# aquaskyline/SOAPdenovo-Trans

Measured on AMD Instinct MI355X. Metric: pregraph k-mers hashed/sec, higher is better.
Workload: dtype u64

## Files before the change

### soapdenovo-trans_amd/csrc/sdt_sk_scatter_seq.cuh

```cuda
#pragma once
#include <hip/hip_runtime.h>
#include "sdt_kmer.cuh"
#include "sdt_table.cuh"
#include "sdt_superkmer.cuh"

using namespace sdt;

constexpr uint32_t SK_BLK = 128;
#ifndef SDT_SK_BLK2
#define SDT_SK_BLK2 1024
#endif
constexpr uint32_t SK_BLK2 = SDT_SK_BLK2;
constexpr uint32_t SK_DEAD = 0xFFFFFFFFu;

#ifdef SDT_SK_L2_LOG
extern __device__ unsigned long long *g_l2_log;
extern __device__ unsigned long long g_l2_log_cap;
__device__ inline void sk_log_alloc(uint32_t path, uint32_t end, uint32_t id)
{
	if (g_l2_log) {
		const unsigned long long at = atomicAdd(g_l2_log, 1ULL);
		if (at + 1 < g_l2_log_cap)
			g_l2_log[1 + at] = (1ULL << 63) | ((unsigned long long)path << 61) | ((unsigned long long)(threadIdx.x & 0x1FFF) << 48) |
			                   ((unsigned long long)(end & 0xFFFFFFu) << 24) | (unsigned long long)(id & 0xFFFFFFu);
	}
}
__device__ inline void sk_log_cursor(uint32_t kind, uint32_t lb, uint32_t chunk, uint32_t pos)
{
	if (g_l2_log) {
		const unsigned long long at = atomicAdd(g_l2_log, 1ULL);
		if (at + 1 < g_l2_log_cap)
			g_l2_log[1 + at] = (1ULL << 63) | (3ULL << 61) | ((unsigned long long)kind << 59) | ((unsigned long long)(blockIdx.x & 15u) << 55) |
			                   ((unsigned long long)(threadIdx.x & 1023u) << 45) | ((unsigned long long)(lb & 1023u) << 35) |
			                   ((unsigned long long)(pos > 31u ? 31u : pos) << 30) | (unsigned long long)(chunk & 0x3FFFFFFFu);
	}
}
#else
__device__ inline void sk_log_alloc(uint32_t, uint32_t, uint32_t) {}
__device__ inline void sk_log_cursor(uint32_t, uint32_t, uint32_t, uint32_t) {}
#endif

__device__ inline uint32_t sk_alloc_chunk(unsigned long long *s_blk, const SkPool &pool, uint32_t blk = SK_BLK)
{
	uint32_t got = 0;
	bool done = false;
	while (!done) {
		{
			const unsigned long long w = __hip_atomic_load(s_blk, __ATOMIC_RELAXED, __HIP_MEMORY_SCOPE_WORKGROUP);
			if ((uint32_t)w > (uint32_t)(w >> 32)) {
				__builtin_amdgcn_s_sleep(1);
				continue;
			}
		}
		const unsigned long long v = atomicAdd(s_blk, 1ULL);
		const uint32_t id = (uint32_t)v, end = (uint32_t)(v >> 32);
		if (id < end) {
			got = id;
			done = true;
			sk_log_alloc(0, end, id);
		} else if (id == end) {
			const uint32_t base = atomicAdd(pool.next, blk);
			atomicExch(s_blk, ((unsigned long long)(base + blk) << 32) | (unsigned long long)(base + 1u));
			got = base;
			done = true;
			sk_log_alloc(1, end, base);
		}
	}
	return got;
}

__device__ inline uint32_t sk_alloc_chunks(unsigned long long *s_blk, const SkPool &pool, uint32_t n, uint32_t blk)
{
	uint32_t got = SK_NOCHUNK;
	bool done = false;
	while (!done) {
		{
			const unsigned long long w = __hip_atomic_load(s_blk, __ATOMIC_RELAXED, __HIP_MEMORY_SCOPE_WORKGROUP);
			if ((uint32_t)w > (uint32_t)(w >> 32)) {
				__builtin_amdgcn_s_sleep(1);
				continue;
			}
		}
		const unsigned long long v = atomicAdd(s_blk, (unsigned long long)n);
		const uint32_t id = (uint32_t)v, end = (uint32_t)(v >> 32);
		if (id <= end && id + n <= end) {
			got = id;
			done = true;
		} else if (id <= end) {
			for (uint32_t x = id; x < end && x < pool.chunks; x++)
				pool.meta[x] = SK_DEAD;
			const uint32_t base = atomicAdd(pool.next, n + blk);
			atomicExch(s_blk, ((unsigned long long)(base + n + blk) << 32) | (unsigned long long)(base + n));
			got = base;
			done = true;
		}
	}
	return got;
}

__device__ inline void sk_retire_block(unsigned long long blk, const SkPool &pool)
{
	const uint32_t next = (uint32_t)blk, end = (uint32_t)(blk >> 32);
	for (uint32_t id = next; id < end && id < pool.chunks; id++)
		pool.meta[id] = SK_DEAD;
}

__device__ inline bool sk_reserve(unsigned long long *s_cur, unsigned long long *s_blk, uint32_t lb, uint32_t meta_bucket,
                                  uint32_t cap, const SkPool &pool, uint32_t *s_cnt, uint32_t &chunk, uint32_t &pos)
{
	bool done = false, ok = false;
	while (!done) {
		if ((uint32_t)__hip_atomic_load(&s_cur[lb], __ATOMIC_RELAXED, __HIP_MEMORY_SCOPE_WORKGROUP) > cap) {
			__builtin_amdgcn_s_sleep(1);
			continue;
		}
		const unsigned long long cur = atomicAdd(&s_cur[lb], 1ULL);
		pos = (uint32_t)cur;
		chunk = (uint32_t)(cur >> 32);
		if (pos < cap) {
			ok = chunk != SK_NOCHUNK;
			done = true;
			sk_log_cursor(0, lb, chunk, pos);
		} else if (pos == cap) {
			sk_log_cursor(1, lb, chunk, pos);
			uint32_t id = sk_alloc_chunk(s_blk, pool);
			if (id >= pool.chunks) {
				id = SK_NOCHUNK;
			} else {
				pool.meta[id] = meta_bucket | (cap << 24);
				atomicAdd(&s_cnt[lb], 1u);
			}
			atomicExch(&s_cur[lb], ((unsigned long long)id << 32) | 1ULL);
			chunk = id;
			pos = 0;
			ok = id != SK_NOCHUNK;
			done = true;
			sk_log_cursor(3, lb, id, 1);
		} else {
#if SDT_SK_L2_LOG >= 2
			sk_log_cursor(2, lb, chunk, pos);
#endif
		}
	}
	return ok;
}

template <int RW> __device__ inline void sk_store_record(uint64_t *dst, const uint64_t (&rec)[RW])
{
#pragma unroll
	for (int i = 0; i < RW; i++)
		dst[i] = rec[i];
}
template <int NW> __device__ inline void sk_store_record2(uint64_t *dst, const uint64_t (&rec)[SkFmt<NW>::REC_WORDS])
{
	if constexpr (SkFmt<NW>::REC2_STRIDE == 4 && SkFmt<NW>::REC_WORDS == 3) {
		ulonglong2 *d = reinterpret_cast<ulonglong2 *>(dst);
		d[0] = make_ulonglong2(rec[0], rec[1]);
		d[1] = make_ulonglong2(rec[2], 0ULL);
	} else {
		sk_store_record<SkFmt<NW>::REC_WORDS>(dst, rec);
	}
}
template <int RW> __device__ inline void sk_load_record(const uint64_t *src, uint64_t (&rec)[RW])
{
#pragma unroll
	for (int i = 0; i < RW; i++)
		rec[i] = src[i];
}


constexpr int SK_SEQ_TILE = 256;
constexpr int SK_SEQ_RUNCAP = 24;
constexpr int SK_SEQ_MAX_KMERS = 256;


template <int NW>
__device__ inline void sk_emit_run(const uint32_t *words, int rb_r, int len_r, int nk_r, int K, uint64_t read_ord, int j0, int n,
                                   uint32_t fb, unsigned long long *s_cur, unsigned long long *s_blk, const SkPool &pool,
                                   uint32_t *s_cnt, const Table<NW> &tbl, uint32_t &claimed, uint32_t &failed, uint32_t &done,
                                   uint32_t &emitted)
{
	constexpr int BW = SkFmt<NW>::BW, RW = SkFmt<NW>::REC_WORDS;
	const int hp = j0 > 0, hn = j0 + n < nk_r;
	const uint32_t l1 = fb >> SK_L2BITS, l2 = fb & (SK_NB2 - 1);
	uint32_t chunk, pos;
	if (sk_reserve(s_cur, s_blk, l1, l1, SK_CAP1, pool, s_cnt, chunk, pos)) {
		const int len = hp + n + K - 1 + hn, ps = rb_r + j0 - hp;
		uint64_t rec[RW];
		rec[0] = sk_header(read_ord, (uint32_t)j0, l2, n, hp, hn);
#pragma unroll
		for (int k = 0; k < BW; k++) {
			uint64_t wv = 0;
			if (32 * k < len) {
				wv = sk_stream_word(words, ps + 32 * k);
				const int keep = len - 32 * k;
				if (keep < 32)
					wv &= ~0ULL << (64 - 2 * keep);
			}
			rec[1 + k] = wv;
		}
		sk_store_record<RW>(pool.recs + ((size_t)chunk * SK_CAP1 + pos) * RW, rec);
		emitted += (uint32_t)n;
	} else if (!tbl.ent) {
		failed += (uint32_t)n;
	} else {
		for (int jj = j0; jj < j0 + n; jj++) {
			uint32_t prev, next;
			const Key<NW> key = chop_record<NW>(words, rb_r, len_r, jj, K, prev, next);
			const uint64_t ord = tbl.first ? (read_ord << 16) | (uint64_t)jj : ORD_NONE;
			if (!table_put<NW>(tbl, key, prev, next, claimed, ord))
				failed++;
			done++;
		}
	}
}

template <int NW, int W>
__global__ __launch_bounds__(SK_SEQ_TILE, NW == 1 ? 4 : 2) void k_sk_scatter_reads_seq(const uint32_t *__restrict__ packed, const uint64_t *__restrict__ offs,
                                                                      uint64_t nreads, int K, int m, int ncap, int max_tile_words, SkPool pool,
                                                                      unsigned long long *__restrict__ g_cursors, unsigned long long *__restrict__ g_blk,
                                                                      uint32_t *__restrict__ g_cnt, Table<NW> tbl, Stats *stats,
                                                                      uint64_t ord_base, uint64_t ord_stride)
{
	constexpr int TR = SK_SEQ_TILE;
	extern __shared__ uint32_t smem[];
	unsigned long long *s_cur = (unsigned long long *)smem;
	uint32_t *s_rb = (uint32_t *)(s_cur + SK_NB1);
	uint32_t *s_runs = s_rb + TR + 2;
	uint32_t *s_words = s_runs + TR * SK_SEQ_RUNCAP;
	__shared__ unsigned long long s_blk;
	__shared__ uint32_t s_cnt[SK_NB1];
	const int tid = threadIdx.x;
	for (int i = tid; i < SK_NB1; i += TR) {
		s_cur[i] = g_cursors[(size_t)blockIdx.x * SK_NB1 + i];
		s_cnt[i] = 0;
	}
	if (tid == 0)
		s_blk = g_blk[blockIdx.x];
	const uint64_t ntiles = (nreads + TR - 1) / TR;
	const uint32_t mmask = (1u << (2 * m)) - 1u;
	const int topsh = 2 * (m - 1);
	uint32_t claimed = 0, failed = 0, done = 0, emitted = 0;
#ifdef SDT_SK_TICKS
	unsigned long long cyc[4] = {0, 0, 0, 0}, t0 = wall_clock64(), t1;
#define SK_TICK(i) do { t1 = wall_clock64(); cyc[i] += t1 - t0; t0 = t1; } while (0)
#else
#define SK_TICK(i) do { } while (0)
#endif
	for (uint64_t tile = blockIdx.x; tile < ntiles; tile += gridDim.x) {
		const uint64_t r0 = tile * TR;
		const int nr = (int)((nreads - r0) < (uint64_t)TR ? (nreads - r0) : (uint64_t)TR);
		const uint64_t word0 = offs[r0] >> 4;
		int nwords = (int)(((offs[r0 + nr] + 15) >> 4) - word0) + TAIL_PAD;
		if (nwords > max_tile_words)
			nwords = max_tile_words;
		s_rb[tid] = (uint32_t)(offs[r0 + (tid < nr ? tid : nr)] - (word0 << 4));
		if (tid == 0)
			s_rb[TR] = (uint32_t)(offs[r0 + nr] - (word0 << 4));
		if (tid < LDS_LEAD)
			s_words[tid] = 0;
		for (int i = tid; i < nwords; i += TR)
			s_words[LDS_LEAD + i] = packed[word0 + i];
		__syncthreads();
		SK_TICK(0);
		const uint32_t *words = s_words + LDS_LEAD;
		const int rb_r = (int)s_rb[tid];
		const int len_r = tid < nr ? (int)s_rb[tid + 1] - rb_r : 0;
		const int nk_r = len_r >= K + 1 ? len_r - K + 1 : 0;
		const uint64_t read_ord = ord_base + (r0 + (uint64_t)tid) * ord_stride;
		uint32_t *runs = s_runs + tid * SK_SEQ_RUNCAP;
		int nrun = 0;
		if (nk_r > 0) {
			const int nhv = len_r - m + 1;
			uint32_t fw = sk_stream_mmer(words, rb_r, m) >> 2;
			uint32_t rc = (sk_rev2bit32(fw ^ 0xAAAAAAAAu) >> (32 - 2 * (m - 1))) << 2;
			int pb = rb_r + m - 1;
			auto next_hv = [&]() -> uint32_t {
				const uint32_t b = (words[pb >> 4] >> (30 - 2 * (pb & 15))) & 3u;
				pb++;
				fw = ((fw << 2) | b) & mmask;
				rc = (rc >> 2) | ((b ^ 2u) << topsh);
				return sk_mmer_hash(fw < rc ? fw : rc);
			};
			int j0 = 0;
			uint32_t fb0 = 0, pfb = 0;
			auto window = [&](int j, uint32_t mn) {
				const uint32_t fb = sk_final_bucket(sk_bucket_hash(mn));
				if (j == 0) {
					fb0 = fb;
				} else if (j - j0 >= ncap || fb != pfb) {
					if (nrun < SK_SEQ_RUNCAP)
						runs[nrun] = (fb0 << 6) | (uint32_t)(j - j0 - 1);
					else
						sk_emit_run<NW>(words, rb_r, len_r, nk_r, K, read_ord, j0, j - j0, fb0, s_cur, &s_blk, pool, s_cnt, tbl, claimed, failed, done, emitted);
					nrun++;
					j0 = j;
					fb0 = fb;
				}
				pfb = fb;
			};
			uint32_t h[W], nh[W];
#pragma clang loop unroll(full)
			for (int i = 0; i < W; i++)
				h[i] = next_hv();
#pragma clang loop unroll(full)
			for (int i = W - 2; i >= 0; i--)
				h[i] = h[i] < h[i + 1] ? h[i] : h[i + 1];
			int p = W;
			for (int jb = 0; jb < nk_r; jb += W) {
				window(jb, h[0]);
				uint32_t pre = 0xFFFFFFFFu;
#pragma clang loop unroll(full)
				for (int i = 1; i < W; i++) {
					const uint32_t x = p < nhv ? next_hv() : 0xFFFFFFFFu;
					p++;
					nh[i - 1] = x;
					pre = x < pre ? x : pre;
					if (jb + i < nk_r)
						window(jb + i, h[i] < pre ? h[i] : pre);
				}
				nh[W - 1] = p < nhv ? next_hv() : 0xFFFFFFFFu;
				p++;
				h[W - 1] = nh[W - 1];
#pragma clang loop unroll(full)
				for (int i = W - 2; i >= 0; i--)
					h[i] = nh[i] < h[i + 1] ? nh[i] : h[i + 1];
			}
			if (nrun < SK_SEQ_RUNCAP)
				runs[nrun] = (fb0 << 6) | (uint32_t)(nk_r - j0 - 1);
			else
				sk_emit_run<NW>(words, rb_r, len_r, nk_r, K, read_ord, j0, nk_r - j0, fb0, s_cur, &s_blk, pool, s_cnt, tbl, claimed, failed, done, emitted);
			nrun++;
		}
		SK_TICK(1);
		const int nlist = nrun < SK_SEQ_RUNCAP ? nrun : SK_SEQ_RUNCAP;
		for (int k = 0, jr = 0; k < nlist; k++) {
			const uint32_t e = runs[k];
			const int nr = (int)(e & 63u) + 1;
			sk_emit_run<NW>(words, rb_r, len_r, nk_r, K, read_ord, jr, nr, e >> 6, s_cur, &s_blk, pool, s_cnt, tbl, claimed, failed, done, emitted);
			jr += nr;
		}
		__syncthreads();
		SK_TICK(3);
	}
#undef SK_TICK
	for (int i = tid; i < SK_NB1; i += TR) {
		g_cursors[(size_t)blockIdx.x * SK_NB1 + i] = s_cur[i];
		if (s_cnt[i])
			atomicAdd(&g_cnt[i], s_cnt[i]);
	}
	if (tid == 0) {
		g_blk[blockIdx.x] = s_blk;
#ifdef SDT_SK_TICKS
		for (int i = 0; i < 4; i++)
			atomicAdd(&stats->sk_cyc1[i], cyc[i]);
#endif
	}
	if (done) {
		atomicAdd(&stats->kmers, (unsigned long long)done);
		atomicAdd(&stats->sk_direct, (unsigned long long)done);
	}
	if (claimed) atomicAdd(&stats->distinct, (unsigned long long)claimed);
	if (failed) atomicAdd(&stats->probe_fail, (unsigned long long)failed);
#pragma unroll
	for (int d = 32; d > 0; d >>= 1)
		emitted += __shfl_down(emitted, d);
	if ((tid & 63) == 0 && emitted)
		atomicAdd(&stats->sk_emitted, (unsigned long long)emitted);
}


struct SkSeqLaunch {
	const uint32_t *words;
	const uint64_t *offs;
	uint64_t nreads;
	int K, m, ncap, mtw;
	SkPool pool;
	unsigned long long *cursors, *blk;
	uint32_t *cnt;
	Stats *stats;
	uint64_t ord_base, ord_stride;
	unsigned max_wgs;
	int cu_count;
	hipStream_t stream;
};

template <int NW, int W> inline hipError_t sk_seq_launch_one(const SkSeqLaunch &a, const Table<NW> &tbl)
{
	const size_t smem = (size_t)SK_NB1 * 8 + (size_t)(SK_SEQ_TILE + 2) * 4 + (size_t)SK_SEQ_TILE * SK_SEQ_RUNCAP * 4 + (size_t)(LDS_LEAD + a.mtw) * 4;
	hipError_t e = hipFuncSetAttribute((const void *)k_sk_scatter_reads_seq<NW, W>, hipFuncAttributeMaxDynamicSharedMemorySize, (int)smem);
	if (e != hipSuccess) return e;
	int per_cu = 0;
	e = hipOccupancyMaxActiveBlocksPerMultiprocessor(&per_cu, k_sk_scatter_reads_seq<NW, W>, SK_SEQ_TILE, smem);
	if (e != hipSuccess) return e;
	uint64_t res = (uint64_t)(per_cu > 0 ? per_cu : 1) * (uint64_t)a.cu_count;
	if (res > a.max_wgs) res = a.max_wgs;
	const uint64_t nt = (a.nreads + SK_SEQ_TILE - 1) / SK_SEQ_TILE;
	const unsigned grid = (unsigned)(nt < res ? nt : res);
	hipLaunchKernelGGL((k_sk_scatter_reads_seq<NW, W>), dim3(grid), dim3(SK_SEQ_TILE), smem, a.stream, a.words, a.offs, a.nreads, a.K, a.m, a.ncap,
	                   a.mtw, a.pool, a.cursors, a.blk, a.cnt, tbl, a.stats, a.ord_base, a.ord_stride);
	return hipGetLastError();
}

hipError_t sk_seq_launch_nw1(int w, const SkSeqLaunch &a, const Table<1> &tbl);
hipError_t sk_seq_launch_nw2_lo(int w, const SkSeqLaunch &a, const Table<2> &tbl);
hipError_t sk_seq_launch_nw2_mid(int w, const SkSeqLaunch &a, const Table<2> &tbl);
hipError_t sk_seq_launch_nw2_hi(int w, const SkSeqLaunch &a, const Table<2> &tbl);
```

Before: 95.24 billion.

## Restructure super-k-mer walk with batched base loads and branchless run recording

Moves the minimizer window walk into a reusable helper that loads W bases at once from two LDS words per 16 bases, instead of one LDS read per base. Run boundaries are recorded branchlessly into an LDS list with an extra overflow slot, and a read is re-walked in segments when the list fills, rather than emitting overflow runs inline. The record packing in sk_emit_run now builds 32-bit halves from clamped word loads with masks, replacing the per-word stream-and-branch code. The extra per-thread LDS slot raises shared memory use and could lower occupancy, and the restart logic adds complexity for reads with many runs.

```diff
diff --git a/soapdenovo-trans_amd/csrc/sdt_sk_scatter_seq.cuh b/soapdenovo-trans_amd/csrc/sdt_sk_scatter_seq.cuh
--- a/soapdenovo-trans_amd/csrc/sdt_sk_scatter_seq.cuh
+++ b/soapdenovo-trans_amd/csrc/sdt_sk_scatter_seq.cuh
@@ -174,6 +174,116 @@
 constexpr int SK_SEQ_MAX_KMERS = 256;
 
 
+template <int W, class List>
+__host__ __device__ inline int sk_walk_list(const uint32_t *words, int rb, int nk, int m, int ncap, List &list)
+{
+	constexpr int NA = (W + 15) / 16, CAP = List::CAP;
+	const uint32_t mmask = (1u << (2 * m)) - 1u;
+	const int topsh = 2 * (m - 1);
+	const int ncm1 = ncap - 1;
+	uint32_t fw = sk_stream_mmer(words, rb, m) >> 2;
+	uint32_t rc = (sk_rev2bit32(fw ^ 0xAAAAAAAAu) >> (32 - 2 * (m - 1))) << 2;
+	int pb = rb + m - 1;
+	uint32_t a[NA], c[NA];
+	auto load = [&]() {
+		const int wi = pb >> 4, sh = 32 - 2 * (pb & 15);
+		uint32_t d[NA + 1];
+#pragma clang loop unroll(full)
+		for (int i = 0; i <= NA; i++)
+			d[i] = words[wi + i];
+#pragma clang loop unroll(full)
+		for (int i = 0; i < NA; i++) {
+			a[i] = (uint32_t)((((uint64_t)d[i] << 32) | d[i + 1]) >> sh);
+			c[i] = a[i] ^ 0xAAAAAAAAu;
+		}
+		pb += W;
+	};
+	auto hv = [&](int k) -> uint32_t {
+		const uint32_t b = (a[k >> 4] >> (30 - 2 * (k & 15))) & 3u;
+		const uint32_t bc = (c[k >> 4] >> (30 - 2 * (k & 15))) & 3u;
+		fw = ((fw << 2) | b) & mmask;
+		rc = (rc >> 2) | (bc << topsh);
+		return sk_mmer_hash(fw < rc ? fw : rc);
+	};
+	uint32_t h[W], nh[W];
+	load();
+#pragma clang loop unroll(full)
+	for (int i = 0; i < W; i++)
+		h[i] = hv(i);
+#pragma clang loop unroll(full)
+	for (int i = W - 2; i >= 0; i--)
+		h[i] = h[i] < h[i + 1] ? h[i] : h[i + 1];
+	int nm1 = -1, nrun = 0;
+	uint32_t pfb = sk_final_bucket(sk_bucket_hash(h[0]));
+	auto window = [&](uint32_t mn) {
+		const uint32_t fb = sk_final_bucket(sk_bucket_hash(mn));
+		const bool end = nm1 >= ncm1 || fb != pfb;
+		list.put(nrun < CAP ? nrun : CAP, (pfb << 6) | (uint32_t)nm1);
+		nrun += end ? 1 : 0;
+		nm1 = end ? 0 : nm1 + 1;
+		pfb = fb;
+	};
+	for (int jb = 0; jb < nk && nrun < CAP; jb += W) {
+		const int nv = nk - jb;
+		uint32_t pre = 0xFFFFFFFFu;
+		if (nv > W) {
+			load();
+			window(h[0]);
+#pragma clang loop unroll(full)
+			for (int i = 1; i < W; i++) {
+				const uint32_t x = hv(i - 1);
+				nh[i - 1] = x;
+				pre = x < pre ? x : pre;
+				window(h[i] < pre ? h[i] : pre);
+			}
+			nh[W - 1] = hv(W - 1);
+			h[W - 1] = nh[W - 1];
+#pragma clang loop unroll(full)
+			for (int i = W - 2; i >= 0; i--)
+				h[i] = nh[i] < h[i + 1] ? nh[i] : h[i + 1];
+		} else {
+			if (nv > 1)
+				load();
+			window(h[0]);
+#pragma clang loop unroll(full)
+			for (int i = 1; i < W; i++) {
+				if (i < nv) {
+					const uint32_t x = hv(i - 1);
+					pre = x < pre ? x : pre;
+					window(h[i] < pre ? h[i] : pre);
+				}
+			}
+		}
+	}
+	list.put(nrun < CAP ? nrun : CAP, (pfb << 6) | (uint32_t)nm1);
+	nrun++;
+	return nrun < CAP ? nrun : CAP;
+}
+
+template <int W, class List, class Run, class Tick>
+__host__ __device__ inline void sk_walk_read(const uint32_t *words, int rb, int nk, int m, int ncap, List &list, Run &&run, Tick &&tick)
+{
+	int js = 0;
+	do {
+		const int nl = sk_walk_list<W>(words, rb + js, nk - js, m, ncap, list);
+		tick(1);
+		for (int k = 0; k < nl; k++) {
+			const uint32_t e = list.get(k);
+			const int n = (int)(e & 63u) + 1;
+			run(js, n, e >> 6);
+			js += n;
+		}
+		tick(3);
+	} while (js < nk);
+}
+
+struct SkLdsRuns {
+	static constexpr int CAP = SK_SEQ_RUNCAP;
+	uint32_t *p;
+	__device__ inline void put(int slot, uint32_t e) { p[slot] = e; }
+	__device__ inline uint32_t get(int slot) const { return p[slot]; }
+};
+
 template <int NW>
 __device__ inline void sk_emit_run(const uint32_t *words, int rb_r, int len_r, int nk_r, int K, uint64_t read_ord, int j0, int n,
                                    uint32_t fb, unsigned long long *s_cur, unsigned long long *s_blk, const SkPool &pool,
@@ -188,17 +298,20 @@
 		const int len = hp + n + K - 1 + hn, ps = rb_r + j0 - hp;
 		uint64_t rec[RW];
 		rec[0] = sk_header(read_ord, (uint32_t)j0, l2, n, hp, hn);
-#pragma unroll
-		for (int k = 0; k < BW; k++) {
-			uint64_t wv = 0;
-			if (32 * k < len) {
-				wv = sk_stream_word(words, ps + 32 * k);
-				const int keep = len - 32 * k;
-				if (keep < 32)
-					wv &= ~0ULL << (64 - 2 * keep);
-			}
-			rec[1 + k] = wv;
-		}
+		const int wi = ps >> 4, wl = (ps + len - 1) >> 4, sh = 32 - 2 * (ps & 15);
+		uint32_t d[2 * BW + 1], w[2 * BW];
+#pragma unroll
+		for (int i = 0; i <= 2 * BW; i++)
+			d[i] = words[wi + i < wl ? wi + i : wl];
+#pragma unroll
+		for (int i = 0; i < 2 * BW; i++) {
+			int keep2 = 2 * len - 32 * i;
+			keep2 = keep2 < 0 ? 0 : (keep2 > 32 ? 32 : keep2);
+			w[i] = (uint32_t)((((uint64_t)d[i] << 32) | d[i + 1]) >> sh) & (uint32_t)(0xFFFFFFFF00000000ULL >> keep2);
+		}
+#pragma unroll
+		for (int k = 0; k < BW; k++)
+			rec[1 + k] = ((uint64_t)w[2 * k] << 32) | w[2 * k + 1];
 		sk_store_record<RW>(pool.recs + ((size_t)chunk * SK_CAP1 + pos) * RW, rec);
 		emitted += (uint32_t)n;
 	} else if (!tbl.ent) {
@@ -227,7 +340,7 @@
 	unsigned long long *s_cur = (unsigned long long *)smem;
 	uint32_t *s_rb = (uint32_t *)(s_cur + SK_NB1);
 	uint32_t *s_runs = s_rb + TR + 2;
-	uint32_t *s_words = s_runs + TR * SK_SEQ_RUNCAP;
+	uint32_t *s_words = s_runs + TR * (SK_SEQ_RUNCAP + 1);
 	__shared__ unsigned long long s_blk;
 	__shared__ uint32_t s_cnt[SK_NB1];
 	const int tid = threadIdx.x;
@@ -238,8 +351,6 @@
 	if (tid == 0)
 		s_blk = g_blk[blockIdx.x];
 	const uint64_t ntiles = (nreads + TR - 1) / TR;
-	const uint32_t mmask = (1u << (2 * m)) - 1u;
-	const int topsh = 2 * (m - 1);
 	uint32_t claimed = 0, failed = 0, done = 0, emitted = 0;
 #ifdef SDT_SK_TICKS
 	unsigned long long cyc[4] = {0, 0, 0, 0}, t0 = wall_clock64(), t1;
@@ -268,77 +379,13 @@
 		const int len_r = tid < nr ? (int)s_rb[tid + 1] - rb_r : 0;
 		const int nk_r = len_r >= K + 1 ? len_r - K + 1 : 0;
 		const uint64_t read_ord = ord_base + (r0 + (uint64_t)tid) * ord_stride;
-		uint32_t *runs = s_runs + tid * SK_SEQ_RUNCAP;
-		int nrun = 0;
+		SkLdsRuns list{s_runs + tid * (SK_SEQ_RUNCAP + 1)};
 		if (nk_r > 0) {
-			const int nhv = len_r - m + 1;
-			uint32_t fw = sk_stream_mmer(words, rb_r, m) >> 2;
-			uint32_t rc = (sk_rev2bit32(fw ^ 0xAAAAAAAAu) >> (32 - 2 * (m - 1))) << 2;
-			int pb = rb_r + m - 1;
-			auto next_hv = [&]() -> uint32_t {
-				const uint32_t b = (words[pb >> 4] >> (30 - 2 * (pb & 15))) & 3u;
-				pb++;
-				fw = ((fw << 2) | b) & mmask;
-				rc = (rc >> 2) | ((b ^ 2u) << topsh);
-				return sk_mmer_hash(fw < rc ? fw : rc);
-			};
-			int j0 = 0;
-			uint32_t fb0 = 0, pfb = 0;
-			auto window = [&](int j, uint32_t mn) {
-				const uint32_t fb = sk_final_bucket(sk_bucket_hash(mn));
-				if (j == 0) {
-					fb0 = fb;
-				} else if (j - j0 >= ncap || fb != pfb) {
-					if (nrun < SK_SEQ_RUNCAP)
-						runs[nrun] = (fb0 << 6) | (uint32_t)(j - j0 - 1);
-					else
-						sk_emit_run<NW>(words, rb_r, len_r, nk_r, K, read_ord, j0, j - j0, fb0, s_cur, &s_blk, pool, s_cnt, tbl, claimed, failed, done, emitted);
-					nrun++;
-					j0 = j;
-					fb0 = fb;
-				}
-				pfb = fb;
-			};
-			uint32_t h[W], nh[W];
-#pragma clang loop unroll(full)
-			for (int i = 0; i < W; i++)
-				h[i] = next_hv();
-#pragma clang loop unroll(full)
-			for (int i = W - 2; i >= 0; i--)
-				h[i] = h[i] < h[i + 1] ? h[i] : h[i + 1];
-			int p = W;
-			for (int jb = 0; jb < nk_r; jb += W) {
-				window(jb, h[0]);
-				uint32_t pre = 0xFFFFFFFFu;
-#pragma clang loop unroll(full)
-				for (int i = 1; i < W; i++) {
-					const uint32_t x = p < nhv ? next_hv() : 0xFFFFFFFFu;
-					p++;
-					nh[i - 1] = x;
-					pre = x < pre ? x : pre;
-					if (jb + i < nk_r)
-						window(jb + i, h[i] < pre ? h[i] : pre);
-				}
-				nh[W - 1] = p < nhv ? next_hv() : 0xFFFFFFFFu;
-				p++;
-				h[W - 1] = nh[W - 1];
-#pragma clang loop unroll(full)
-				for (int i = W - 2; i >= 0; i--)
-					h[i] = nh[i] < h[i + 1] ? nh[i] : h[i + 1];
-			}
-			if (nrun < SK_SEQ_RUNCAP)
-				runs[nrun] = (fb0 << 6) | (uint32_t)(nk_r - j0 - 1);
-			else
-				sk_emit_run<NW>(words, rb_r, len_r, nk_r, K, read_ord, j0, nk_r - j0, fb0, s_cur, &s_blk, pool, s_cnt, tbl, claimed, failed, done, emitted);
-			nrun++;
-		}
-		SK_TICK(1);
-		const int nlist = nrun < SK_SEQ_RUNCAP ? nrun : SK_SEQ_RUNCAP;
-		for (int k = 0, jr = 0; k < nlist; k++) {
-			const uint32_t e = runs[k];
-			const int nr = (int)(e & 63u) + 1;
-			sk_emit_run<NW>(words, rb_r, len_r, nk_r, K, read_ord, jr, nr, e >> 6, s_cur, &s_blk, pool, s_cnt, tbl, claimed, failed, done, emitted);
-			jr += nr;
+			sk_walk_read<W>(words, rb_r, nk_r, m, ncap, list,
+			                [&](int j0, int n, uint32_t fb) {
+				                sk_emit_run<NW>(words, rb_r, len_r, nk_r, K, read_ord, j0, n, fb, s_cur, &s_blk, pool, s_cnt, tbl, claimed, failed, done, emitted);
+			                },
+			                [&](int i) { SK_TICK(i); });
 		}
 		__syncthreads();
 		SK_TICK(3);
@@ -387,7 +434,7 @@
 
 template <int NW, int W> inline hipError_t sk_seq_launch_one(const SkSeqLaunch &a, const Table<NW> &tbl)
 {
-	const size_t smem = (size_t)SK_NB1 * 8 + (size_t)(SK_SEQ_TILE + 2) * 4 + (size_t)SK_SEQ_TILE * SK_SEQ_RUNCAP * 4 + (size_t)(LDS_LEAD + a.mtw) * 4;
+	const size_t smem = (size_t)SK_NB1 * 8 + (size_t)(SK_SEQ_TILE + 2) * 4 + (size_t)SK_SEQ_TILE * (SK_SEQ_RUNCAP + 1) * 4 + (size_t)(LDS_LEAD + a.mtw) * 4;
 	hipError_t e = hipFuncSetAttribute((const void *)k_sk_scatter_reads_seq<NW, W>, hipFuncAttributeMaxDynamicSharedMemorySize, (int)smem);
 	if (e != hipSuccess) return e;
 	int per_cu = 0;
```

Result: no change. 97.24 billion, median of 6 (+2.1%).
